# temudschin/xfemm

Measured on AMD Instinct MI355X. Metric: solved DoF/s (assembly+CG to tol) on 2M-tri magnetostatic, higher is better.
Workload: dtype f64; 1 GPU; configs[2]: synthetic 2000000-tri square-domain magnetostatic, linear mu, tol 1e-08; triangles=2000000, dof_total=1002001, dof_per_gpu=1002001, nnz=7006001, pcg_iters=18, newton_iters=1, pcg=Chronopoulos-Gear + AMG V-cycle, parallelism=single GPU

## Files before the change

### xfemm_amd/csrc/xfk_amg.h

```cpp
#pragma once

#include <hip/hip_runtime.h>

#include <map>
#include <memory>
#include <vector>

#include "xfk_internal.h"
#include "xfk_partition.h"

struct xfk_comm;

namespace xfk {

constexpr int kAmgDenseMax = 2048;
constexpr int kAmgMaxLevels = 16;
constexpr int kAmgDeferSlots = 64;
constexpr int kAmgDeferTotal = kAmgDeferSlots + kAmgDeferSlots / 2;

struct AmgLevel {
    int n = 0;
    long long nnz = 0;
    int ncol_lim = 0;
    int ncol_smooth = 0;
    const int *rowptr = nullptr, *col = nullptr;
    const double *val = nullptr;
    DBuf<int> rowptr_o, col_o;
    DBuf<double> val_o;
    DBuf<double> dinv;
    int nc = 0;
    long long pnnz = 0;
    DBuf<int> prow, pcol, rrow, rcol;
    DBuf<double> pval, rval;
// ... 70 lines not shown
    DBuf<int> cnt, agg1, agg, flag, cursor;
    DBuf<int> ap_row, ap_col;
    DBuf<int> pad_col;
    DBuf<double> pad_val;
    DBuf<double> ap_val;
    DBuf<int> dev_int;
    std::map<int, int> cap_hint;
    std::map<int, int> mis_hint;
    int row_max0 = 0;
    void seed_hints();
    DBuf<int> def_dev;
    int *def_host = nullptr;
    int def_n = 0;
    long long *def_target[kAmgDeferSlots / 2] = {};
    int def_verify[kAmgDeferSlots / 2] = {};
    bool foreign = false;
    std::vector<char> nd_plan;
    size_t nd_tl_n = 0, nd_mask_n = 0;
    int load_hints(hipStream_t s, int n0, long long nnz0);
    void save_hints(int n0, long long nnz0);
    int *host_int = nullptr;
    hipEvent_t ev_host = nullptr;
    DBuf<int> mis_out;
    DBuf<char> cub_tmp;

    bool dist = false;
    int rep_rows = 250000;
    int dense_max = kAmgDenseMax;
    int fold_on = -1;
    int col16 = -1;
    int prec32 = -1;
    int lrep = 0;
    xfk_comm *comm = nullptr;
    int nranks = 1, rank = 0;
    std::vector<int> c0;
    int ncmax = 0;
// ... 10 lines not shown
    int *host_big = nullptr;
    int host_big_n = 0;
    double *part_gam_ = nullptr;
    SideStream side;
    bool time_tail = false;
    std::vector<hipEvent_t> tail_ev;
    std::vector<char> tail_kind;
    int tail_used = 0;
    int tail_begin(hipStream_t s, int kind);
    void tail_end(hipStream_t s, int at);
    int tail_read(double &ms_cycle, int &cycles, double &ms_setup);
    SideStream sw;
    bool sw_used = false, rt_pending = false, fold_pending = false;
    DBuf<int> cnt2;
    DBuf<char> cub_tmp2;

    ~Amg();
    void sync_streams()
    {
        if (side.cs) (void)hipStreamSynchronize(side.cs);
        if (sw.cs) (void)hipStreamSynchronize(sw.cs);
    }
    int setup(hipStream_t s, int n, int ncol_lim, const int *rowptr, const int *col, const double *val,
              long long nnz);
    int setup_dist(hipStream_t s, xfk_comm *comm, const HaloPlan &halo, int n, int nh, const int *rowptr,
                   const int *col, const double *val, long long nnz);
    int vcycle(hipStream_t s, const double *r, double *u, const int *done, double *part_gam = nullptr);
    bool gamma_done = false;
    int refresh(hipStream_t s, bool fold = true);
    int reserve_host();
// ... 21 lines not shown
```

### xfemm_amd/csrc/xfk_amg.hip

```cpp
#include <hipcub/hipcub.hpp>

#include <algorithm>
#include <climits>
#include <cmath>
#include <cstdio>
#include <cstdlib>
#include <cstring>
#include <map>
#include <mutex>
#include <vector>

#include "xfk_amg.h"
#include "xfk_comm.h"
#include "xfk_spmv.h"

namespace xfk {

namespace {


constexpr int kB = 256;
inline int nb(long long n) { return (int)((n + kB - 1) / kB); }

using MisKey = unsigned;
// ... 316 lines not shown
        *undecided = 1;
    }
    if (ROOTS) flag[i] = root;
}


__global__ void k_mis_pack(const int *__restrict__ roots, const int *__restrict__ und, const int *__restrict__ run,
                           int *__restrict__ out)
{
    if (threadIdx.x == 0) {
        out[0] = *roots;
        out[1] = *und;
        out[2] = *run;
    }
}

__global__ void k_pattern_diff(int n, const int *__restrict__ rowptr, const int *__restrict__ col,
                               const int *__restrict__ key, int key_nnz, int *__restrict__ out)
{
    const int t = blockIdx.x * blockDim.x + threadIdx.x;
    bool d = false;
    if (t <= n) d = rowptr[t] != key[t];
    if (t < key_nnz) d = d || col[t] != key[n + 1 + t];
    if (d) out[0] = 1;
}

template <int G>
__device__ __forceinline__ void join_best_key(MisKey &best, int &bk, int &bj)
{
#pragma unroll
// ... 826 lines not shown
        if (l == 0) M[(size_t)q * ld + q] = 1.0;
        return;
    }
    const double sq = sc[q];
    for (int k = rowptr[i] + l; k < rowptr[i + 1]; k += kDsG) {
        const int cj = col[k];
        if (cj >= n) continue;
        const int c = perm ? perm[cj] : cj;
        M[(size_t)q * ld + c] = 0.0 + val[k] * sq * sc[c];
    }
}

template <class V>
__global__ void __launch_bounds__(256) k_dense_unperm(int n, int ld, int ldo, const double *__restrict__ M,
                                                      const double *__restrict__ sc, const int *__restrict__ iperm,
                                                      V *__restrict__ out, double *__restrict__ osc)
{
    __shared__ double t[64][65];
    const int bq = blockIdx.y * 64, br = blockIdx.x * 64;
    for (int k = threadIdx.x; k < 64 * 64; k += 256) {
        const int a = k & 63, b = k >> 6;
        t[a][b] = M[(size_t)(br + b) * ld + bq + a];
    }
    __syncthreads();
    for (int k = threadIdx.x; k < 64 * 64; k += 256) {
        const int a = k >> 6, b = k & 63, q = bq + a, r = br + b;
        const int i = iperm ? iperm[q] : (q < n ? q : -1), j = iperm ? iperm[r] : (r < n ? r : -1);
        if (i >= 0 && j >= 0) out[(size_t)i * ldo + j] = (V)(0.5 * (M[(size_t)q * ld + r] + t[a][b]));
    }
    if (blockIdx.x == 0)
        for (int a = threadIdx.x; a < 64; a += 256) {
            const int q = bq + a, i = iperm ? iperm[q] : (q < n ? q : -1);
            if (i >= 0) osc[i] = sc[q];
        }
// ... 1255 lines not shown
        int *slot = M.def_dev.p + M.def_n;
        int *need = (verify && cap > 16) ? M.def_dev.p + kAmgDeferSlots + M.def_n / 2 : nullptr;
        M.def_verify[M.def_n / 2] = need ? cap : 0;
        AMG_CHECK(M.pad_col.alloc((size_t)nrows * cap));
        AMG_CHECK(M.pad_val.alloc((size_t)nrows * cap));
        AMG_CHECK(ccol.alloc((size_t)std::max(1LL, (long long)nrows * cap)));
        AMG_CHECK(cval.alloc((size_t)std::max(1LL, (long long)nrows * cap)));
        launch_sort(cap, slot, need);
        int rc = scan_only(M, s, M.cnt.p, crow.p, nrows);
        if (rc != XFK_OK) return rc;
        if (nrows > 0)
            launch_compact(s, nrows, cap, crow.p, slab_n, M.pad_col.p, M.pad_val.p, ccol.p, cval.p, slot + 1);
        else
            AMG_CHECK(hipMemsetAsync(slot + 1, 0, sizeof(int), s));
        M.def_target[M.def_n / 2] = &cnnz;
        M.def_n += 2;
        cnnz = (long long)nrows * cap;
        return XFK_OK;
    };
    if (key >= 0) {
        auto hint = M.cap_hint.find(key);
        if (hint != M.cap_hint.end()) {
            if (defer && M.def_n + 2 <= kAmgDeferSlots) return deferred_pass(hint->second, M.foreign);
            if (M.foreign) {
                M.cap_hint.erase(hint);
                hint = M.cap_hint.end();
            }
        }
        if (hint != M.cap_hint.end()) {
            bool overflow = false;
// ... 374 lines not shown
    static const bool v = [] {
        const char *e = std::getenv("XFK_NO_SPEC");
        return !(e && std::atoi(e) != 0);
    }();
    return v;
}

bool overlap_enabled()
{
    const char *n = std::getenv("XFK_NO_OVERLAP");
    if (n && std::atoi(n) != 0) return false;
    const char *e = std::getenv("XFK_OVERLAP");
    return e && std::atoi(e) != 0;
}

int Amg::resolve_deferred(hipStream_t s, bool &overflow)
{
    int rc = fetch_deferred(s);
    if (rc != XFK_OK) return rc;
    return wait_deferred(s, overflow);
}

int Amg::fetch_deferred(hipStream_t s)
{
    if (def_n == 0) return XFK_OK;
    AMG_CHECK(hipMemcpyAsync(def_host, def_dev.p, sizeof(int) * kAmgDeferTotal, hipMemcpyDeviceToHost, s));
    AMG_CHECK(hipEventRecord(ev_host, s));
    return XFK_OK;
}

int Amg::wait_deferred(hipStream_t s, bool &overflow)
{
    overflow = false;
    if (def_n == 0) return XFK_OK;
    AMG_CHECK(hipEventSynchronize(ev_host));
    for (int q = 0; q < def_n / 2; ++q) {
        if (def_host[2 * q]) overflow = true;
        else if (def_verify[q] && !def_host[kAmgDeferSlots + q]) overflow = true;
        else *def_target[q] = def_host[2 * q + 1];
        def_verify[q] = 0;
    }
    def_n = 0;
    AMG_CHECK(hipMemsetAsync(def_dev.p, 0, sizeof(int) * kAmgDeferTotal, s));
    return XFK_OK;
}

int Amg::host_ints(int count)
{
    if (host_big_n >= count) return XFK_OK;
    pinned_free(host_big);
    host_big = nullptr;
    host_big_n = 0;
    AMG_CHECK(pinned_malloc((void **)&host_big, sizeof(int) * std::max(count, 1)));
    host_big_n = count;
    return XFK_OK;
}

int Amg::reserve_host()
// ... 8 lines not shown
    }
    constexpr size_t kStage = 64 << 10;
    if (nd_stage_n < kStage) {
        pinned_free(nd_stage);
        nd_stage = nullptr;
        nd_stage_n = 0;
        AMG_CHECK(pinned_malloc((void **)&nd_stage, kStage));
        nd_stage_n = kStage;
    }
    return XFK_OK;
}

int Amg::init(hipStream_t s)
{
    if (!host_int) AMG_CHECK(pinned_malloc((void **)&host_int, 16 * sizeof(int)));
    if (!ev_host) AMG_CHECK(hipEventCreateWithFlags(&ev_host, hipEventDisableTiming));
    if (!def_host) AMG_CHECK(pinned_malloc((void **)&def_host, kAmgDeferTotal * sizeof(int)));
    AMG_CHECK(dev_int.alloc(8));
    AMG_CHECK(def_dev.alloc(kAmgDeferTotal));
    def_n = 0;
    for (int &v : def_verify) v = 0;
    AMG_CHECK(rho.alloc(2 * kAmgMaxLevels));
    k_setup_zero<<<1, 64, 0, s>>>(def_dev.p, kAmgDeferTotal, rho.p, 2 * kAmgMaxLevels);
    if (L.empty()) L.emplace_back(new AmgLevel());
    for (auto &lv : L) {
        lv->dist = false;
        lv->has16 = false;
        lv->has32 = false;
        lv->plan = HaloPlan();
        lv->ts.B = 0;
// ... 154 lines not shown
        save_hints(n0, nnz0);
    }
    return rc;
}

static bool rt_tile_on()
{
    static const bool v = [] {
        const char *e = std::getenv("XFK_RT_TILE");
        return !(e && std::atoi(e) == 0);
    }();
    return v;
}

static int transpose_csr(DBuf<int> &cnt, DBuf<char> &tmp, hipStream_t s, int n, int nc, const int *mrow,
                         const int *mcol, const double *mval, int *trow, int *tcol, double *tval)
{
    AMG_CHECK(cnt.alloc((size_t)std::max(n, nc) + 1));
    AMG_CHECK(hipMemsetAsync(cnt.p, 0, sizeof(int) * ((size_t)nc + 1), s));
    const bool tiled = rt_tile_on();
    if (n > 0) {
        if (tiled) k_rt_tile<false><<<nb(n), 256, 0, s>>>(n, mrow, mcol, mval, trow, cnt.p, tcol, tval);
        else k_rt_count<<<nb(n), kB, 0, s>>>(n, mrow, mcol, cnt.p);
    }
    int rc = scan_only(tmp, s, cnt.p, trow, nc);
    if (rc != XFK_OK) return rc;
    if (tiled) {
        if (n > 0) k_rt_tile<true><<<nb(n), 256, 0, s>>>(n, mrow, mcol, mval, trow, cnt.p, tcol, tval);
        if (nc > 0) k_rt_sort_pairs<<<(int)((((long long)nc + 3) / 4 * 64 + 255) / 256), 256, 0, s>>>(nc, trow, tcol, tval);
        AMG_CHECK(hipGetLastError());
        return XFK_OK;
    }
    if (n > 0) k_rt_fill<<<nb(n), kB, 0, s>>>(n, mrow, mcol, trow, cnt.p, tcol);
    if (nc > 0)
        k_rt_sort_vals<<<(int)(((long long)nc * 64 + 255) / 256), 256, 0, s>>>(nc, trow, tcol, mrow, mcol, mval, tval);
    AMG_CHECK(hipGetLastError());
    return XFK_OK;
}

template <int B>
static int build_col16(hipStream_t st, int n, const int *rowptr, const int *col, long long nnz,
                       DBuf<unsigned short> &c16, DBuf<int> &base)
{
    const int nt = (n + B - 1) / B;
    AMG_CHECK(c16.alloc((size_t)std::max(1LL, nnz)));
    AMG_CHECK(base.alloc((size_t)std::max(1, nt)));
    if (nt > 0) k_tile_col16<B><<<nt, 256, 0, st>>>(n, rowptr, col, c16.p, base.p);
// ... 39 lines not shown
                else
                    k_mis_update<4><<<nb(4LL * n), kB, 0, s>>>(n, A.rowptr, cv, sflag.p, t1.p, key.p, prev, cur,
                                                                nullptr, xc);
            } else {
                k_mis_max<1><<<nb(n), kB, 0, s>>>(n, A.rowptr, cv, sflag.p, key.p, t1.p, prev, cur, run, act.p, xc);
                if (last)
                    k_mis_update<1, true><<<nb(n), kB, 0, s>>>(n, A.rowptr, cv, sflag.p, t1.p, key.p, prev, cur,
                                                                flag.p, xc);
                else
                    k_mis_update<1><<<nb(n), kB, 0, s>>>(n, A.rowptr, cv, sflag.p, t1.p, key.p, prev, cur, nullptr,
                                                          xc);
            }
        }
        int rc = scan_only(*this, s, flag.p, cursor.p, n);
        if (rc != XFK_OK) return rc;
        k_mis_pack<<<1, 64, 0, s>>>(cursor.p + n, und2 + ((rounds - 1) & 1), run, mis_out.p);
        AMG_CHECK(hipMemcpyAsync(host_int + 8, mis_out.p, 3 * sizeof(int), hipMemcpyDeviceToHost, s));
        AMG_CHECK(hipEventRecord(ev_host, s));
        joined = spec;
        if (spec && (rc = joins_and_p()) != XFK_OK) return rc;
        AMG_CHECK(hipEventSynchronize(ev_host));
        if (!host_int[9]) break;
        joined = false;
        if (rounds > 4096) {
            set_error("AMG: MIS-2 aggregation did not terminate");
            return XFK_ERR_NOCONV;
        }
    }
    mis_hint[l] = host_int[10];
    nc = host_int[8];
    stats.mis_rounds[l] = host_int[10];
    int rc = XFK_OK;
// ... 5 lines not shown
    A.nc = (int)nc;
    if (std::getenv("XFK_AMG_DEBUG")) std::fprintf(stderr, "[amg] level %d P nnz %lld\n", l, A.pnnz);
    AMG_CHECK(A.rrow.alloc((size_t)nc + 1));
    AMG_CHECK(A.rcol.alloc((size_t)std::max(1LL, A.pnnz)));
    AMG_CHECK(A.rval.alloc((size_t)std::max(1LL, A.pnnz)));
    const bool off = side_setup_on() && !A.dist && !dist;
    hipStream_t ts = s;
    if (off) {
        if ((rc = sw.init()) != XFK_OK) return rc;
        AMG_CHECK(hipEventRecord(sw.a, s));
        AMG_CHECK(hipStreamWaitEvent(sw.cs, sw.a, 0));
        ts = sw.cs;
        sw_used = true;
    }
    if ((rc = transpose_csr(off ? cnt2 : cnt, off ? cub_tmp2 : cub_tmp, ts, n, (int)nc, A.prow.p, A.pcol.p,
                            A.pval.p, A.rrow.p, A.rcol.p, A.rval.p)) != XFK_OK)
        return rc;
    if (off) {
        AMG_CHECK(hipEventRecord(sw.b, sw.cs));
        rt_pending = true;
    }
    if (l == 0 && A.has16 && (rc = build_col16<256>(ts, (int)nc, A.rrow.p, A.rcol.p, A.pnnz, A.r16, A.r16b)) != XFK_OK)
        return rc;
    if (l == 0 && A.has32 &&
        ((rc = to_f32(ts, (int)nc, A.rrow.p, A.pnnz, A.rval.p, A.r32)) != XFK_OK ||
         (f32_sweep_on() && (rc = to_f32(ts, n, A.rowptr, A.nnz, A.val, A.a32)) != XFK_OK)))
        return rc;
    if (l == 0 && A.has32 && A.dist &&
        ((rc = to_f32(ts, n, A.prow.p, A.pnnz, A.pval.p, A.p32)) != XFK_OK ||
         (rc = build_col16<256>(ts, n, A.prow.p, A.pcol.p, A.pnnz, A.p16, A.p16b)) != XFK_OK))
        return rc;
// ... 315 lines not shown
        st.nn = 1;
        st.nx[0] = 0;
        st.Dn[0] = Db(0, 0);
        st.Rn[0] = Rb(0, 0);
        st.Cn[0] = Cb(0, 0);
        k_bgj_init<<<1 + 2 * nbk, 256, 0, s>>>(nbk, ld, cinv.p, st, maxd, bgj_inv_mode());
        for (int k = 0; k < nbk; ++k) {
            const int p = k & 1, q = (k + 1) & 1;
            k_bgj_step<<<nbk * nbk, 256, 0, s>>>(k, nbk, ld, cinv.p, Db(0, p), Rb(0, p), Cb(0, p), Db(0, q),
                                                 Rb(0, q), Cb(0, q), maxd, bgj_inv_mode());
        }
    }
    {
        const int ldo = ((C.n + kBj - 1) / kBj) * kBj;
        const dim3 g(ld / 64, ld / 64);
        AMG_CHECK(cinv_sc.alloc((size_t)ldo));
        cinv_f64 = !(prec32 < 0 ? f32_on() : prec32 != 0);
        if (cinv_f64) {
            AMG_CHECK(cinv_o64.alloc((size_t)ldo * ldo));
            AMG_CHECK(hipMemsetAsync(cinv_o64.p, 0, sizeof(double) * (size_t)ldo * ldo, s));
            k_dense_unperm<double><<<g, 256, 0, s>>>(C.n, ld, ldo, cinv.p, sc, nd ? cinv_iperm.p : nullptr,
                                                     cinv_o64.p, cinv_sc.p);
        } else {
            AMG_CHECK(cinv_o.alloc((size_t)ldo * ldo));
            AMG_CHECK(hipMemsetAsync(cinv_o.p, 0, sizeof(float) * (size_t)ldo * ldo, s));
            k_dense_unperm<float><<<g, 256, 0, s>>>(C.n, ld, ldo, cinv.p, sc, nd ? cinv_iperm.p : nullptr, cinv_o.p,
                                                    cinv_sc.p);
        }
        cinv_apply = cinv_o.p;
        cinv_ld = ldo;
    }
    return XFK_OK;
}

int Amg::alloc_vectors()
{
    for (int k = 0; k < nlev; ++k) {
        AmgLevel &A = *L[k];
        const size_t nv = (size_t)std::max(1, std::max(A.n, A.ncol_smooth));
        AMG_CHECK(A.xa.alloc(nv));
        AMG_CHECK(A.xb.alloc(nv));
        AMG_CHECK(A.r.alloc((size_t)std::max(1, A.n)));
// ... 39 lines not shown
        k_max_reduce<<<1, kMaxReduceT, 0, s>>>(nb_str(n), rho_part.p, omega, rho.p + 2 * l);
        if (g_prof) g_prof->end();
        if (l == kAmgMaxLevels - 1) break;
        long long nc = 0;
        int rc = aggregate(s, l, nc, true);
        if (rc != XFK_OK) return rc;
        if (nc == 0) break;
        SgX XA{A.rowptr, A.col, A.val, A.ncol_lim, nullptr, nullptr, nullptr, A.has16 ? A.a16.p : nullptr,
               A.has16 ? A.a16b.p : nullptr};
        SgY YP{A.prow.p, A.pcol.p, A.pval.p, nullptr};
        if (fold_pending) {
            AMG_CHECK(hipStreamWaitEvent(s, sw.c, 0));
            fold_pending = false;
        }
        if (g_prof) g_prof->begin(lv + "SpGEMM A P", 0.0);
        rc = spgemm<false>(*this, s, n, XA, YP, A.ftrow, ap_col, ap_val, ap_nnz, 4 * l + 1);
        if (g_prof) g_prof->end();
        if (rc != XFK_OK) return rc;
        if ((int)L.size() <= l + 1) L.emplace_back(new AmgLevel());
        AmgLevel &C = *L[l + 1];
        SgX XR{A.rrow.p, A.rcol.p, A.rval.p, INT_MAX, nullptr, nullptr, nullptr};
        SgY YAP{A.ftrow.p, ap_col.p, ap_val.p, nullptr};
        if (rt_pending) {
            AMG_CHECK(hipStreamWaitEvent(s, sw.b, 0));
            rt_pending = false;
        }
        if (g_prof) g_prof->begin(lv + "SpGEMM R (A P)", 0.0);
        rc = spgemm<false>(*this, s, (int)nc, XR, YAP, C.rowptr_o, C.col_o, C.val_o, C.nnz, 4 * l + 2);
        if (g_prof) g_prof->end();
        if (rc != XFK_OK) return rc;
        A.fold = (fold_on < 0 ? fold_levels() : fold_on != 0) && sweeps == 1 && !A.dist;
// ... 20 lines not shown
            }
            if (n > 0)
                k_fold_p<<<(int)(((long long)n * kFoldLanes + 255) / 256), 256, 0, fs>>>(
                    n, rho.p + 2 * l, A.dinv.p, A.ftrow.p, ap_col.p, ap_val.p, A.prow.p, A.pcol.p, A.pval.p, A.ftcol.p,
                    A.ftval.p);
            if (l == 0 && A.has16 &&
                (rc = build_col16<kCgBlock>(fs, n, A.ftrow.p, A.ftcol.p, ap_nnz, A.f16, A.f16b)) != XFK_OK)
                return rc;
            if (l == 0 && A.has32 && (rc = to_f32(fs, n, A.ftrow.p, ap_nnz, A.ftval.p, A.f32v)) != XFK_OK) return rc;
            if (off) {
                AMG_CHECK(hipEventRecord(sw.c, sw.cs));
                fold_pending = true;
            }
            if (l > 0)
                rc = transpose_csr(off ? cnt2 : cnt, off ? cub_tmp2 : cub_tmp, fs, n, (int)nc, A.ftrow.p, A.ftcol.p,
                                   A.ftval.p, A.frrow.p, A.frcol.p, A.frval.p);
            if (rc != XFK_OK) return rc;
            if (def_n > 0 && def_n + 2 <= kAmgDeferSlots) {
                AMG_CHECK(hipMemcpyAsync(def_dev.p + def_n + 1, A.ftrow.p + n, sizeof(int), hipMemcpyDeviceToDevice, s));
                def_target[def_n / 2] = &A.fnnz;
                def_n += 2;
            } else if (def_n > 0) {
                int len = 0;
                AMG_CHECK(hipMemcpyAsync(&len, A.ftrow.p + n, sizeof(int), hipMemcpyDeviceToHost, s));
                AMG_CHECK(hipStreamSynchronize(s));
                A.fnnz = len;
            }
            if (g_prof) g_prof->end();
        }
        C.n = (int)nc;
        C.ncol_lim = (int)nc;
        C.ncol_smooth = (int)nc;
        C.rowptr = C.rowptr_o.p;
        C.col = C.col_o.p;
        C.val = C.val_o.p;
    }
    nlev = l + 1;
    {
        AmgLevel &C = *L[nlev - 1];
        const bool nd_spec = dense_coarse && spec_on() && !g_prof && def_n > 0 && nlev - 1 > l0 &&
                             C.n >= 8 * kBj && nd_key_n == C.n && C.col == C.col_o.p &&
                             (size_t)nd_key_nnz <= C.col_o.n && !std::getenv("XFK_NO_ND");
        if (nd_spec) {
            AMG_CHECK(mis_out.alloc(4));
            AMG_CHECK(hipMemsetAsync(mis_out.p + 3, 0, sizeof(int), s));
            const int nt = (int)std::max((long long)C.n + 1, nd_key_nnz);
            k_pattern_diff<<<nb(nt), kB, 0, s>>>(C.n, C.rowptr, C.col, nd_key_dev.p, (int)nd_key_nnz, mis_out.p + 3);
            AMG_CHECK(hipMemcpyAsync(host_int + 11, mis_out.p + 3, sizeof(int), hipMemcpyDeviceToHost, s));
        }
        int rc = fetch_deferred(s);
        if (rc != XFK_OK) return rc;
        if (nd_spec) {
            rc = alloc_vectors();
            if (rc != XFK_OK) return rc;
            nd_phases = nd_phases_key;
            if ((rc = dense_inverse(s, C, nd_ld)) != XFK_OK) return rc;
        }
        bool overflow = false;
        rc = wait_deferred(s, overflow);
        if (rc != XFK_OK) return rc;
        if (overflow) {
            if (sw_used) {
                AMG_CHECK(hipStreamSynchronize(sw.cs));
                sw_used = rt_pending = fold_pending = false;
            }
            cap_hint.clear();
            return build(s, l0);
        }
        for (int k = l0; k < nlev; ++k) stats.nnz[k] = L[k]->nnz;
        if (std::getenv("XFK_AMG_HINTS_PRINT")) {
            std::fprintf(stderr, "[amg hints] levels %d:", nlev);
            for (auto &h : cap_hint) std::fprintf(stderr, " cap[%d.%d]=%d", h.first / 4, h.first % 4, h.second);
            for (auto &h : mis_hint) std::fprintf(stderr, " mis[%d]=%d", h.first, h.second);
            for (int k = 0; k < nlev; ++k) std::fprintf(stderr, " n%d=%d/%lld", k, L[k]->n, L[k]->nnz);
            std::fprintf(stderr, "\n");
// ... 893 lines not shown
```

### xfemm_amd/csrc/xfk_api.hip

```cpp
#include <hipcub/hipcub.hpp>

#include "xfk_amg.h"
#include "xfk_spmv.h"

#include <algorithm>
#include <atomic>
#include <chrono>
#include <cmath>
#include <cstring>
#include <map>
#include <mutex>
#include <iterator>
#include <set>
#include <type_traits>
#include <unordered_map>

#include "xfk_age.h"
#include "xfk_comm.h"
#include "xfk_kernels.h"
#include "xfk_magdir.h"
#include <cstdio>
#include <cstdlib>
#include "xfk_partition.h"

// ... 817 lines not shown
        void *tmp = nullptr;
        size_t bytes = 0;
        XFK_CHECK(hipcub::DeviceRadixSort::SortPairs(tmp, bytes, P->color.p, T.keys_out, T.iota, P->perm.p, NE, 0,
                                                     8, s));
        XFK_CHECK(cub_scratch(P, bytes, &tmp));
        XFK_CHECK(hipcub::DeviceRadixSort::SortPairs(tmp, bytes, P->color.p, T.keys_out, T.iota, P->perm.p, NE, 0,
                                                     8, s));
    }
    XFK_CHECK(P->erec.alloc(NE));
    XFK_CHECK(P->ebits.alloc(NE));
    XFK_CHECK(P->slot.alloc(9 * (size_t)NE));
    launch_build_erec(s, NE, P->perm.p, P->p_raw.p, P->lbl_raw.p, P->ebits_raw.p, P->erec.p, P->ebits.p, T.iperm);
    launch_build_slots(s, NE, N, P->p_raw.p, T.iperm, P->rowptr.p, P->col.p, P->slot.p, T.cnt);
    }

    launch_mark_fix_adj(s, N, P->rowptr.p, P->col.p, P->fixed.p, T.flag);
    XFK_CHECK(P->fix_cols_row.alloc(N));
    launch_compact_flags(s, N, T.flag, T.cnt + 1, P->fix_cols_row.p);
    if (P->harmonic) {
        XFK_CHECK(hipMemcpyAsync(P->hpin + 2, T.cnt, sizeof(int) * 2, hipMemcpyDeviceToHost, s));
        XFK_CHECK(hipStreamSynchronize(s));
        const int hc[2] = {P->hpin[2], P->hpin[3]};
        XFK_REQUIRE(hc[0] == 0, XFK_ERR_HIP, "internal: element slot missing from the CSR pattern");
        P->nfix_cols = hc[1];
    } else {
        XFK_CHECK(P->nfix_dev.alloc(1));
        XFK_CHECK(hipMemcpyAsync(P->nfix_dev.p, T.cnt + 1, sizeof(int), hipMemcpyDeviceToDevice, s));
        P->nfix_cols = -1;
    }
    XFK_CHECK(P->mu1.alloc(NE));
    XFK_CHECK(P->mu2.alloc(NE));
    if (!P->harmonic) {
        XFK_CHECK(P->mu1b.alloc(NE));
        XFK_CHECK(P->mu2b.alloc(NE));
        if (P->any_nonlinear && !P->axi) {
            XFK_CHECK(P->dv_el.alloc(NE));
            XFK_CHECK(P->on_el.alloc(NE));
        }
        XFK_CHECK(P->asm_miss.alloc(1));
        XFK_CHECK(hipMemsetAsync(P->asm_miss.p, 0, sizeof(int), s));
        P->miss_checked = false;
    }

    P->age_n = 0;
    if (!P->age_key.empty()) {
        std::vector<int> rc;
        std::vector<double> v;
        for (size_t m = 0; m < P->age_key.size(); ++m) {
            const int r = (int)(P->age_key[m] >> 32), c = (int)(P->age_key[m] & 0xffffffff);
            rc.push_back(r); rc.push_back(c); v.push_back(P->age_val[m]);
            if (r != c) { rc.push_back(c); rc.push_back(r); v.push_back(P->age_val[m]); }
        }
        const int na = (int)v.size();
        DBuf<int> d_rc;
        XFK_CHECK(upload(d_rc, rc.data(), rc.size(), s));
// ... 98 lines not shown
        XFK_CHECK(upload(P->pa_ptr, ptr.data(), ptr.size(), s));
        XFK_CHECK(upload(P->pa_w, w.data(), w.size(), s));
        XFK_CHECK(P->pa_tmp.alloc(nd));
        std::vector<int> chk(nd), chk2(ns);
        XFK_CHECK(d2h(chk.data(), P->pa_dst.p, sizeof(int) * nd, s));
        if (ns) XFK_CHECK(d2h(chk2.data(), P->pa_src.p, sizeof(int) * ns, s));
        for (int v : chk) XFK_REQUIRE(v >= 0, XFK_ERR_HIP, "internal: auxiliary periodic map slot missing");
        for (int v : chk2) XFK_REQUIRE(v >= 0, XFK_ERR_HIP, "internal: auxiliary periodic map source slot missing");
        P->pa_n = nd;
    }

    for (DBuf<double> *v : {&P->b, &P->P, &P->dinv}) XFK_CHECK(v->alloc(N));
    for (DBuf<double> *v : {&P->V, &P->Vold}) XFK_CHECK(v->alloc(NL));
    XFK_CHECK(P->partials.alloc(2 * kRedGrid));
    XFK_CHECK(P->counters.alloc(8));
    XFK_CHECK(hipMemsetAsync(P->counters.p, 0, sizeof(unsigned) * 8, s));
    XFK_CHECK(P->pcg.alloc(1));
    XFK_CHECK(P->nws.alloc(1));
    int rc2 = alloc_cg(P);
    if (rc2 != XFK_OK) return rc2;
    P->symbolic_ready = true;
    return XFK_OK;
}

static int assemble(xfk_problem *P, int iter)
{
    hipStream_t s = P->stream;
    AssembleArgs A = {};
    A.erec = P->erec.p;
    A.ebits = P->ebits.p;
    A.slot = P->slot.p;
// ... 1889 lines not shown
```

### xfemm_amd/csrc/xfk_device.hip

```cpp
#include "xfk_kernels.h"
#include "xfk_axi.h"
#include "xfk_spmv.h"

namespace xfk {


__device__ __forceinline__ double wave_sum(double v)
{
#pragma unroll
    for (int off = 32; off > 0; off >>= 1) v += __shfl_xor(v, off, 64);
    return v;
}

__device__ __forceinline__ double block_sum(double v, double *lds)
{
    v = wave_sum(v);
    const int lane = threadIdx.x & 63, wid = threadIdx.x >> 6;
    __syncthreads();
    if (lane == 0) lds[wid] = v;
    __syncthreads();
    double r = 0.0;
    if (threadIdx.x == 0) {
        const int nw = (blockDim.x + 63) >> 6;
        for (int w = 0; w < nw; ++w) r += lds[w];
// ... 571 lines not shown
            dst[3 * j + q] = s[q];
        }
    }
    if (missing) atomicAdd(bad, 1);
}

__global__ void k_lookup_slots(int n, const int *__restrict__ rc, const int *__restrict__ rowptr,
                               const int *__restrict__ col, int *__restrict__ out)
{
    int i = blockIdx.x * blockDim.x + threadIdx.x;
    if (i >= n) return;
    out[i] = find_slot(rowptr, col, rc[2 * i], rc[2 * i + 1]);
}

__global__ void k_mark_fix_adj(int N, const int *__restrict__ rowptr, const int *__restrict__ col,
                               const unsigned char *__restrict__ fixed, int *__restrict__ flag)
{
    int r = blockIdx.x * blockDim.x + threadIdx.x;
    if (r >= N) return;
    int f = 0;
    if (!fixed[r])
        for (int k = rowptr[r]; k < rowptr[r + 1]; ++k) f |= fixed[col[k]];
    flag[r] = f;
}

__global__ void k_compact_flags(int N, const int *__restrict__ flag, int *__restrict__ cursor,
                                int *__restrict__ out)
{
    int r = blockIdx.x * blockDim.x + threadIdx.x;
    if (r >= N || !flag[r]) return;
    out[atomicAdd(cursor, 1)] = r;
}

// ... 656 lines not shown
void launch_build_erec(hipStream_t s, int NE, const int *perm, const int *p, const int *lbl, const int *ebits_raw,
                       int4 *erec, int *ebits, int *iperm)
{
    if (NE) k_build_erec<<<nblk(NE), kBlock, 0, s>>>(NE, perm, p, lbl, ebits_raw, erec, ebits, iperm);
}
void launch_build_slots(hipStream_t s, int NE, int nrows, const int *p, const int *iperm, const int *rowptr,
                        const int *col, int *slot, int *bad)
{
    if (NE) k_build_slots<<<nblk(NE), kBlock, 0, s>>>(NE, nrows, p, iperm, rowptr, col, slot, bad);
}
void launch_lookup_slots(hipStream_t s, int n, const int *rc, const int *rowptr, const int *col, int *out)
{
    if (n) k_lookup_slots<<<nblk(n), kBlock, 0, s>>>(n, rc, rowptr, col, out);
}
void launch_mark_fix_adj(hipStream_t s, int N, const int *rowptr, const int *col, const unsigned char *fixed,
                         int *flag)
{
    if (N) k_mark_fix_adj<<<nblk(N), kBlock, 0, s>>>(N, rowptr, col, fixed, flag);
}
void launch_compact_flags(hipStream_t s, int N, const int *flag, int *cursor, int *out)
{
    if (N) k_compact_flags<<<nblk(N), kBlock, 0, s>>>(N, flag, cursor, out);
}
void launch_assemble_rows(hipStream_t s, int N, const AssembleArgs &A)
{
    if (N <= 0) return;
    const int g = (N + kRowBlock - 1) / kRowBlock;
    static const bool xcd = [] {
        const char *e = std::getenv("XFK_ASM_XCD");
        return !(e && std::atoi(e) == 0);
    }();
    if (!xcd && !A.axi) {
        if (A.iter == 0) k_assemble_rows<false, true, false><<<g, kRowBlock, 0, s>>>(N, A);
// ... 72 lines not shown
```

### xfemm_amd/csrc/xfk_internal.h

```cpp
#pragma once

#include <hip/hip_runtime.h>

#include <algorithm>
#include <cstdint>
#include <map>
#include <string>
#include <unordered_map>
#include <thread>
#include <vector>

#include "../../include/xfemm_kernels.h"
#include "xfk_partition.h"

struct xfk_comm;

namespace xfk {

struct Amg;

constexpr int kBlock = 256;
constexpr int kRedGrid = 1024;
constexpr double kPI = 3.141592653589793238462643383;
constexpr double kDEG = 0.01745329251994329576923690768;
// ... 225 lines not shown
hipError_t warm_module_postproc();
hipError_t warm_module_sort();
void stream_release(hipStream_t s);
void stream_pool_drain();
int sort_elements_device(hipStream_t s, int n, const unsigned *score_dev, int *perm_dev, unsigned long long *key,
                         unsigned long long *tmp, unsigned long long *red, unsigned long long *cin, int *flag,
                         int *passes);
long long stream_pool_idle();
struct SideStream {
    hipStream_t cs = nullptr;
    hipEvent_t a = nullptr, b = nullptr, c = nullptr;
    int init();
    ~SideStream();
};
bool overlap_enabled();
template <class Ex, class In, class Bd>
int exchange_overlapped(hipStream_t s, SideStream &ss, Ex &&exch, In &&interior, Bd &&boundary)
{
    XFK_CHECK(hipEventRecord(ss.a, s));
    XFK_CHECK(hipStreamWaitEvent(ss.cs, ss.a, 0));
    const int rc = exch(ss.cs);
    if (rc != XFK_OK) return rc;
    XFK_CHECK(hipEventRecord(ss.b, ss.cs));
    interior();
    XFK_CHECK(hipStreamWaitEvent(s, ss.b, 0));
    boundary();
    return XFK_OK;
}

}
// ... 332 lines not shown
```

### xfemm_amd/csrc/xfk_kernels.h

```cpp
#pragma once

#include "xfk_internal.h"

namespace xfk {

struct AssembleArgs {
    const int4 *erec;
    const int *ebits;
    const int *slot;
    const double *x, *y;
    const DevLabel *labels;
    const DevBlock *blocks;
    const DevLine *lines;
    const DevCirc *circs;
    const double *bhB, *bhH, *bhS;
    double *mu1, *mu2;
    const double *V;
    double *val, *b;
    int iter;
    int axi;
    double ext_ro, ext_ri, ext_zo;
    const int *p_raw, *lbl_raw, *ebits_raw, *n2e_ptr, *n2e, *rowptr, *col;
    double *mu1_out, *mu2_out;
    int *miss;
// ... 46 lines not shown
void launch_row_copy(hipStream_t s, int N, const int *p, const int *n2e_ptr, const int *n2e, const int *fill_ptr,
                     const int *fill_col, const int *tmp, const int *rowptr, int *col, int *diag);
void launch_jp_round(hipStream_t s, int N, int NE, int round, unsigned char *active, int *pending_round,
                     const int *p, const int *n2e_ptr, const int *n2e, int *color, unsigned long long *maxkey,
                     unsigned long long *used);
void launch_color_hist(hipStream_t s, int NE, const int *color, int *hist, int maxc);
void launch_iota(hipStream_t s, int n, int *a);
void launch_build_erec(hipStream_t s, int NE, const int *perm, const int *p, const int *lbl, const int *ebits_raw,
                       int4 *erec, int *ebits, int *iperm);
void launch_build_slots(hipStream_t s, int NE, int nrows, const int *p, const int *iperm, const int *rowptr,
                        const int *col, int *slot, int *bad);
void launch_add_at_slots(hipStream_t s, int n, const int *slot, const double *v, double *data);
void launch_lookup_slots(hipStream_t s, int n, const int *rc, const int *rowptr, const int *col, int *out);
void launch_mark_fix_adj(hipStream_t s, int N, const int *rowptr, const int *col, const unsigned char *fixed,
                         int *flag);
void launch_compact_flags(hipStream_t s, int N, const int *flag, int *cursor, int *out);
void launch_assemble_rows(hipStream_t s, int N, const AssembleArgs &A);
void launch_point_currents(hipStream_t s, int n, const int *nodes, const double *J, double *b);
void launch_dirichlet(hipStream_t s, int nrows, const int *rows, int nadj, const int *nadj_dev, int nadj_max,
                      const int *adj, const int *rowptr, const int *col, const int *diag, const unsigned char *fixed,
                      const double *fix_first, const double *fix_last, double *val, double *b);
void launch_map(hipStream_t s, int n, const int *dst, const int *ptr, const int *src, const double *w,
                double *data, double *tmp);
void launch_diag_inv(hipStream_t s, int N, const int *diag, const double *val, double *dinv, CgState *S);
void launch_newton_res(hipStream_t s, int N, const double *V, const double *Vold, double *partials,
                       unsigned *counter, NewtonScalars *S);
void launch_relax(hipStream_t s, int N, double relax, double *V, const double *Vold);
void launch_scale(hipStream_t s, int N, double sc, const double *V, double *out);

}
// ... 1 lines not shown
```

Before: 189.2 million DoF/s.

## Trim memsets and copies from the AMG setup and assembly launch chain

Adds a default-on XFK_LEAN_CHAIN mode that removes small memsets and memcpys from the stream. The MIS pack kernel writes straight into mapped pinned host memory. The pattern-diff flag rides along with the deferred-readback buffer, and the dense-inverse padding is zeroed inside the unpermute kernel instead of a full memset. The transpose counter memset is skipped when the buffer is known clean, deferred fnnz reuses an earlier slot, and the fix-adjacency kernel zeroes the counters. The aim is to cut launch and API overhead in setup, at the cost of relying on buffer-cleanliness invariants that could go stale.

```diff
diff --git a/xfemm_amd/csrc/xfk_amg.h b/xfemm_amd/csrc/xfk_amg.h
--- a/xfemm_amd/csrc/xfk_amg.h
+++ b/xfemm_amd/csrc/xfk_amg.h
@@ -16,7 +16,8 @@
 constexpr int kAmgDenseMax = 2048;
 constexpr int kAmgMaxLevels = 16;
 constexpr int kAmgDeferSlots = 64;
-constexpr int kAmgDeferTotal = kAmgDeferSlots + kAmgDeferSlots / 2;
+constexpr int kAmgDeferNd = kAmgDeferSlots + kAmgDeferSlots / 2;
+constexpr int kAmgDeferTotal = kAmgDeferNd + 1;
 
 struct AmgLevel {
     int n = 0;
@@ -117,12 +118,14 @@
     int def_n = 0;
     long long *def_target[kAmgDeferSlots / 2] = {};
     int def_verify[kAmgDeferSlots / 2] = {};
+    int def_src[kAmgDeferSlots / 2] = {};
     bool foreign = false;
     std::vector<char> nd_plan;
     size_t nd_tl_n = 0, nd_mask_n = 0;
     int load_hints(hipStream_t s, int n0, long long nnz0);
     void save_hints(int n0, long long nnz0);
     int *host_int = nullptr;
+    int *host_int_dev = nullptr;
     hipEvent_t ev_host = nullptr;
     DBuf<int> mis_out;
     DBuf<char> cub_tmp;
@@ -163,6 +166,8 @@
     bool sw_used = false, rt_pending = false, fold_pending = false;
     DBuf<int> cnt2;
     DBuf<char> cub_tmp2;
+    size_t rt_clean = 0;
+    int *rt_clean_p = nullptr;
 
     ~Amg();
     void sync_streams()
diff --git a/xfemm_amd/csrc/xfk_amg.hip b/xfemm_amd/csrc/xfk_amg.hip
--- a/xfemm_amd/csrc/xfk_amg.hip
+++ b/xfemm_amd/csrc/xfk_amg.hip
@@ -354,6 +354,20 @@
         out[2] = *run;
     }
 }
+__global__ void k_mis_pack_host(const int *__restrict__ roots, const int *__restrict__ und,
+                                const int *__restrict__ run, int *__restrict__ out, int *__restrict__ host)
+{
+    if (threadIdx.x == 0) {
+        const int a = *roots, b = *und, c = *run;
+        out[0] = a;
+        out[1] = b;
+        out[2] = c;
+        host[0] = a;
+        host[1] = b;
+        host[2] = c;
+        __threadfence_system();
+    }
+}
 
 __global__ void k_pattern_diff(int n, const int *__restrict__ rowptr, const int *__restrict__ col,
                                const int *__restrict__ key, int key_nnz, int *__restrict__ out)
@@ -1210,10 +1224,18 @@
 template <class V>
 __global__ void __launch_bounds__(256) k_dense_unperm(int n, int ld, int ldo, const double *__restrict__ M,
                                                       const double *__restrict__ sc, const int *__restrict__ iperm,
-                                                      V *__restrict__ out, double *__restrict__ osc)
+                                                      V *__restrict__ out, double *__restrict__ osc, bool pad)
 {
     __shared__ double t[64][65];
     const int bq = blockIdx.y * 64, br = blockIdx.x * 64;
+    if (pad) {
+        const long long np = ldo - n, tot = np * ldo + (long long)n * np;
+        const long long nthr = (long long)gridDim.x * gridDim.y * 256;
+        for (long long k = ((long long)blockIdx.y * gridDim.x + blockIdx.x) * 256 + threadIdx.x; k < tot; k += nthr) {
+            if (k < np * ldo) out[(size_t)n * ldo + k] = (V)0;
+            else out[(size_t)((k - np * ldo) / np) * ldo + n + (k - np * ldo) % np] = (V)0;
+        }
+    }
     for (int k = threadIdx.x; k < 64 * 64; k += 256) {
         const int a = k & 63, b = k >> 6;
         t[a][b] = M[(size_t)(br + b) * ld + bq + a];
@@ -2499,6 +2521,7 @@
         else
             AMG_CHECK(hipMemsetAsync(slot + 1, 0, sizeof(int), s));
         M.def_target[M.def_n / 2] = &cnnz;
+        M.def_src[M.def_n / 2] = M.def_n / 2;
         M.def_n += 2;
         cnnz = (long long)nrows * cap;
         return XFK_OK;
@@ -2903,6 +2926,15 @@
     return e && std::atoi(e) != 0;
 }
 
+bool lean_chain()
+{
+    static const bool v = [] {
+        const char *e = std::getenv("XFK_LEAN_CHAIN");
+        return !(e && std::atoi(e) == 0);
+    }();
+    return v;
+}
+
 int Amg::resolve_deferred(hipStream_t s, bool &overflow)
 {
     int rc = fetch_deferred(s);
@@ -2926,11 +2958,11 @@
     for (int q = 0; q < def_n / 2; ++q) {
         if (def_host[2 * q]) overflow = true;
         else if (def_verify[q] && !def_host[kAmgDeferSlots + q]) overflow = true;
-        else *def_target[q] = def_host[2 * q + 1];
+        else *def_target[q] = def_host[2 * def_src[q] + 1];
         def_verify[q] = 0;
     }
     def_n = 0;
-    AMG_CHECK(hipMemsetAsync(def_dev.p, 0, sizeof(int) * kAmgDeferTotal, s));
+    if (!lean_chain() || overflow) AMG_CHECK(hipMemsetAsync(def_dev.p, 0, sizeof(int) * kAmgDeferTotal, s));
     return XFK_OK;
 }
 
@@ -2969,6 +3001,7 @@
 int Amg::init(hipStream_t s)
 {
     if (!host_int) AMG_CHECK(pinned_malloc((void **)&host_int, 16 * sizeof(int)));
+    if (!host_int_dev) AMG_CHECK(hipHostGetDevicePointer((void **)&host_int_dev, host_int, 0));
     if (!ev_host) AMG_CHECK(hipEventCreateWithFlags(&ev_host, hipEventDisableTiming));
     if (!def_host) AMG_CHECK(pinned_malloc((void **)&def_host, kAmgDeferTotal * sizeof(int)));
     AMG_CHECK(dev_int.alloc(8));
@@ -3153,11 +3186,15 @@
 }
 
 static int transpose_csr(DBuf<int> &cnt, DBuf<char> &tmp, hipStream_t s, int n, int nc, const int *mrow,
-                         const int *mcol, const double *mval, int *trow, int *tcol, double *tval)
+                         const int *mcol, const double *mval, int *trow, int *tcol, double *tval,
+                         size_t *clean = nullptr, int **clean_p = nullptr)
 {
     AMG_CHECK(cnt.alloc((size_t)std::max(n, nc) + 1));
-    AMG_CHECK(hipMemsetAsync(cnt.p, 0, sizeof(int) * ((size_t)nc + 1), s));
     const bool tiled = rt_tile_on();
+    const bool keep = clean && clean_p && *clean_p == cnt.p && *clean >= (size_t)nc + 1;
+    const size_t was = keep ? *clean : 0;
+    if (!keep) AMG_CHECK(hipMemsetAsync(cnt.p, 0, sizeof(int) * ((size_t)nc + 1), s));
+    if (clean) *clean = 0;
     if (n > 0) {
         if (tiled) k_rt_tile<false><<<nb(n), 256, 0, s>>>(n, mrow, mcol, mval, trow, cnt.p, tcol, tval);
         else k_rt_count<<<nb(n), kB, 0, s>>>(n, mrow, mcol, cnt.p);
@@ -3168,8 +3205,13 @@
         if (n > 0) k_rt_tile<true><<<nb(n), 256, 0, s>>>(n, mrow, mcol, mval, trow, cnt.p, tcol, tval);
         if (nc > 0) k_rt_sort_pairs<<<(int)((((long long)nc + 3) / 4 * 64 + 255) / 256), 256, 0, s>>>(nc, trow, tcol, tval);
         AMG_CHECK(hipGetLastError());
+        if (clean) {
+            *clean = std::max(was, (size_t)nc + 1);
+            *clean_p = cnt.p;
+        }
         return XFK_OK;
     }
+    if (clean) *clean = 0;
     if (n > 0) k_rt_fill<<<nb(n), kB, 0, s>>>(n, mrow, mcol, trow, cnt.p, tcol);
     if (nc > 0)
         k_rt_sort_vals<<<(int)(((long long)nc * 64 + 255) / 256), 256, 0, s>>>(nc, trow, tcol, mrow, mcol, mval, tval);
@@ -3239,8 +3281,13 @@
         }
         int rc = scan_only(*this, s, flag.p, cursor.p, n);
         if (rc != XFK_OK) return rc;
-        k_mis_pack<<<1, 64, 0, s>>>(cursor.p + n, und2 + ((rounds - 1) & 1), run, mis_out.p);
-        AMG_CHECK(hipMemcpyAsync(host_int + 8, mis_out.p, 3 * sizeof(int), hipMemcpyDeviceToHost, s));
+        if (lean_chain()) {
+            k_mis_pack_host<<<1, 64, 0, s>>>(cursor.p + n, und2 + ((rounds - 1) & 1), run, mis_out.p,
+                                             host_int_dev + 8);
+        } else {
+            k_mis_pack<<<1, 64, 0, s>>>(cursor.p + n, und2 + ((rounds - 1) & 1), run, mis_out.p);
+            AMG_CHECK(hipMemcpyAsync(host_int + 8, mis_out.p, 3 * sizeof(int), hipMemcpyDeviceToHost, s));
+        }
         AMG_CHECK(hipEventRecord(ev_host, s));
         joined = spec;
         if (spec && (rc = joins_and_p()) != XFK_OK) return rc;
@@ -3276,7 +3323,8 @@
         sw_used = true;
     }
     if ((rc = transpose_csr(off ? cnt2 : cnt, off ? cub_tmp2 : cub_tmp, ts, n, (int)nc, A.prow.p, A.pcol.p,
-                            A.pval.p, A.rrow.p, A.rcol.p, A.rval.p)) != XFK_OK)
+                            A.pval.p, A.rrow.p, A.rcol.p, A.rval.p, off && lean_chain() ? &rt_clean : nullptr,
+                            &rt_clean_p)) != XFK_OK)
         return rc;
     if (off) {
         AMG_CHECK(hipEventRecord(sw.b, sw.cs));
@@ -3622,18 +3670,19 @@
     {
         const int ldo = ((C.n + kBj - 1) / kBj) * kBj;
         const dim3 g(ld / 64, ld / 64);
+        const bool lean = lean_chain();
         AMG_CHECK(cinv_sc.alloc((size_t)ldo));
         cinv_f64 = !(prec32 < 0 ? f32_on() : prec32 != 0);
         if (cinv_f64) {
             AMG_CHECK(cinv_o64.alloc((size_t)ldo * ldo));
-            AMG_CHECK(hipMemsetAsync(cinv_o64.p, 0, sizeof(double) * (size_t)ldo * ldo, s));
+            if (!lean) AMG_CHECK(hipMemsetAsync(cinv_o64.p, 0, sizeof(double) * (size_t)ldo * ldo, s));
             k_dense_unperm<double><<<g, 256, 0, s>>>(C.n, ld, ldo, cinv.p, sc, nd ? cinv_iperm.p : nullptr,
-                                                     cinv_o64.p, cinv_sc.p);
+                                                     cinv_o64.p, cinv_sc.p, lean);
         } else {
             AMG_CHECK(cinv_o.alloc((size_t)ldo * ldo));
-            AMG_CHECK(hipMemsetAsync(cinv_o.p, 0, sizeof(float) * (size_t)ldo * ldo, s));
+            if (!lean) AMG_CHECK(hipMemsetAsync(cinv_o.p, 0, sizeof(float) * (size_t)ldo * ldo, s));
             k_dense_unperm<float><<<g, 256, 0, s>>>(C.n, ld, ldo, cinv.p, sc, nd ? cinv_iperm.p : nullptr, cinv_o.p,
-                                                    cinv_sc.p);
+                                                    cinv_sc.p, lean);
         }
         cinv_apply = cinv_o.p;
         cinv_ld = ldo;
@@ -3703,7 +3752,9 @@
             fold_pending = false;
         }
         if (g_prof) g_prof->begin(lv + "SpGEMM A P", 0.0);
+        const int ap_def = def_n;
         rc = spgemm<false>(*this, s, n, XA, YP, A.ftrow, ap_col, ap_val, ap_nnz, 4 * l + 1);
+        const bool ap_deferred = rc == XFK_OK && def_n == ap_def + 2;
         if (g_prof) g_prof->end();
         if (rc != XFK_OK) return rc;
         if ((int)L.size() <= l + 1) L.emplace_back(new AmgLevel());
@@ -3754,10 +3805,15 @@
             }
             if (l > 0)
                 rc = transpose_csr(off ? cnt2 : cnt, off ? cub_tmp2 : cub_tmp, fs, n, (int)nc, A.ftrow.p, A.ftcol.p,
-                                   A.ftval.p, A.frrow.p, A.frcol.p, A.frval.p);
+                                   A.ftval.p, A.frrow.p, A.frcol.p, A.frval.p,
+                                   off && lean_chain() ? &rt_clean : nullptr, &rt_clean_p);
             if (rc != XFK_OK) return rc;
             if (def_n > 0 && def_n + 2 <= kAmgDeferSlots) {
-                AMG_CHECK(hipMemcpyAsync(def_dev.p + def_n + 1, A.ftrow.p + n, sizeof(int), hipMemcpyDeviceToDevice, s));
+                def_src[def_n / 2] = def_n / 2;
+                if (lean_chain() && ap_deferred) def_src[def_n / 2] = ap_def / 2;
+                else
+                    AMG_CHECK(hipMemcpyAsync(def_dev.p + def_n + 1, A.ftrow.p + n, sizeof(int),
+                                             hipMemcpyDeviceToDevice, s));
                 def_target[def_n / 2] = &A.fnnz;
                 def_n += 2;
             } else if (def_n > 0) {
@@ -3781,12 +3837,18 @@
         const bool nd_spec = dense_coarse && spec_on() && !g_prof && def_n > 0 && nlev - 1 > l0 &&
                              C.n >= 8 * kBj && nd_key_n == C.n && C.col == C.col_o.p &&
                              (size_t)nd_key_nnz <= C.col_o.n && !std::getenv("XFK_NO_ND");
+        const bool lean = lean_chain();
         if (nd_spec) {
-            AMG_CHECK(mis_out.alloc(4));
-            AMG_CHECK(hipMemsetAsync(mis_out.p + 3, 0, sizeof(int), s));
             const int nt = (int)std::max((long long)C.n + 1, nd_key_nnz);
-            k_pattern_diff<<<nb(nt), kB, 0, s>>>(C.n, C.rowptr, C.col, nd_key_dev.p, (int)nd_key_nnz, mis_out.p + 3);
-            AMG_CHECK(hipMemcpyAsync(host_int + 11, mis_out.p + 3, sizeof(int), hipMemcpyDeviceToHost, s));
+            if (lean) {
+                k_pattern_diff<<<nb(nt), kB, 0, s>>>(C.n, C.rowptr, C.col, nd_key_dev.p, (int)nd_key_nnz,
+                                                     def_dev.p + kAmgDeferNd);
+            } else {
+                AMG_CHECK(mis_out.alloc(4));
+                AMG_CHECK(hipMemsetAsync(mis_out.p + 3, 0, sizeof(int), s));
+                k_pattern_diff<<<nb(nt), kB, 0, s>>>(C.n, C.rowptr, C.col, nd_key_dev.p, (int)nd_key_nnz, mis_out.p + 3);
+                AMG_CHECK(hipMemcpyAsync(host_int + 11, mis_out.p + 3, sizeof(int), hipMemcpyDeviceToHost, s));
+            }
         }
         int rc = fetch_deferred(s);
         if (rc != XFK_OK) return rc;
@@ -3799,6 +3861,7 @@
         bool overflow = false;
         rc = wait_deferred(s, overflow);
         if (rc != XFK_OK) return rc;
+        if (nd_spec && lean) host_int[11] = def_host[kAmgDeferNd];
         if (overflow) {
             if (sw_used) {
                 AMG_CHECK(hipStreamSynchronize(sw.cs));
diff --git a/xfemm_amd/csrc/xfk_api.hip b/xfemm_amd/csrc/xfk_api.hip
--- a/xfemm_amd/csrc/xfk_api.hip
+++ b/xfemm_amd/csrc/xfk_api.hip
@@ -855,9 +855,18 @@
     launch_build_slots(s, NE, N, P->p_raw.p, T.iperm, P->rowptr.p, P->col.p, P->slot.p, T.cnt);
     }
 
-    launch_mark_fix_adj(s, N, P->rowptr.p, P->col.p, P->fixed.p, T.flag);
+    const bool lean = lean_chain() && !P->harmonic && N > 0;
+    if (lean) {
+        XFK_CHECK(P->nfix_dev.alloc(1));
+        XFK_CHECK(P->asm_miss.alloc(1));
+        XFK_CHECK(P->counters.alloc(8));
+        launch_mark_fix_adj(s, N, P->rowptr.p, P->col.p, P->fixed.p, T.flag, P->nfix_dev.p, P->asm_miss.p,
+                            P->counters.p);
+    } else {
+        launch_mark_fix_adj(s, N, P->rowptr.p, P->col.p, P->fixed.p, T.flag);
+    }
     XFK_CHECK(P->fix_cols_row.alloc(N));
-    launch_compact_flags(s, N, T.flag, T.cnt + 1, P->fix_cols_row.p);
+    launch_compact_flags(s, N, T.flag, lean ? P->nfix_dev.p : T.cnt + 1, P->fix_cols_row.p);
     if (P->harmonic) {
         XFK_CHECK(hipMemcpyAsync(P->hpin + 2, T.cnt, sizeof(int) * 2, hipMemcpyDeviceToHost, s));
         XFK_CHECK(hipStreamSynchronize(s));
@@ -866,7 +875,7 @@
         P->nfix_cols = hc[1];
     } else {
         XFK_CHECK(P->nfix_dev.alloc(1));
-        XFK_CHECK(hipMemcpyAsync(P->nfix_dev.p, T.cnt + 1, sizeof(int), hipMemcpyDeviceToDevice, s));
+        if (!lean) XFK_CHECK(hipMemcpyAsync(P->nfix_dev.p, T.cnt + 1, sizeof(int), hipMemcpyDeviceToDevice, s));
         P->nfix_cols = -1;
     }
     XFK_CHECK(P->mu1.alloc(NE));
@@ -879,7 +888,7 @@
             XFK_CHECK(P->on_el.alloc(NE));
         }
         XFK_CHECK(P->asm_miss.alloc(1));
-        XFK_CHECK(hipMemsetAsync(P->asm_miss.p, 0, sizeof(int), s));
+        if (!lean) XFK_CHECK(hipMemsetAsync(P->asm_miss.p, 0, sizeof(int), s));
         P->miss_checked = false;
     }
 
@@ -1008,7 +1017,7 @@
     for (DBuf<double> *v : {&P->V, &P->Vold}) XFK_CHECK(v->alloc(NL));
     XFK_CHECK(P->partials.alloc(2 * kRedGrid));
     XFK_CHECK(P->counters.alloc(8));
-    XFK_CHECK(hipMemsetAsync(P->counters.p, 0, sizeof(unsigned) * 8, s));
+    if (!lean) XFK_CHECK(hipMemsetAsync(P->counters.p, 0, sizeof(unsigned) * 8, s));
     XFK_CHECK(P->pcg.alloc(1));
     XFK_CHECK(P->nws.alloc(1));
     int rc2 = alloc_cg(P);
diff --git a/xfemm_amd/csrc/xfk_device.hip b/xfemm_amd/csrc/xfk_device.hip
--- a/xfemm_amd/csrc/xfk_device.hip
+++ b/xfemm_amd/csrc/xfk_device.hip
@@ -609,9 +609,15 @@
 }
 
 __global__ void k_mark_fix_adj(int N, const int *__restrict__ rowptr, const int *__restrict__ col,
-                               const unsigned char *__restrict__ fixed, int *__restrict__ flag)
+                               const unsigned char *__restrict__ fixed, int *__restrict__ flag,
+                               int *__restrict__ z1a, int *__restrict__ z1b, unsigned *__restrict__ z8)
 {
     int r = blockIdx.x * blockDim.x + threadIdx.x;
+    if (blockIdx.x == 0 && threadIdx.x < 8) {
+        if (threadIdx.x == 0 && z1a) *z1a = 0;
+        if (threadIdx.x == 0 && z1b) *z1b = 0;
+        if (z8) z8[threadIdx.x] = 0u;
+    }
     if (r >= N) return;
     int f = 0;
     if (!fixed[r])
@@ -1298,9 +1304,14 @@
     if (n) k_lookup_slots<<<nblk(n), kBlock, 0, s>>>(n, rc, rowptr, col, out);
 }
 void launch_mark_fix_adj(hipStream_t s, int N, const int *rowptr, const int *col, const unsigned char *fixed,
+                         int *flag, int *z1a, int *z1b, unsigned *z8)
+{
+    if (N) k_mark_fix_adj<<<nblk(N), kBlock, 0, s>>>(N, rowptr, col, fixed, flag, z1a, z1b, z8);
+}
+void launch_mark_fix_adj(hipStream_t s, int N, const int *rowptr, const int *col, const unsigned char *fixed,
                          int *flag)
 {
-    if (N) k_mark_fix_adj<<<nblk(N), kBlock, 0, s>>>(N, rowptr, col, fixed, flag);
+    if (N) k_mark_fix_adj<<<nblk(N), kBlock, 0, s>>>(N, rowptr, col, fixed, flag, nullptr, nullptr, nullptr);
 }
 void launch_compact_flags(hipStream_t s, int N, const int *flag, int *cursor, int *out)
 {
diff --git a/xfemm_amd/csrc/xfk_internal.h b/xfemm_amd/csrc/xfk_internal.h
--- a/xfemm_amd/csrc/xfk_internal.h
+++ b/xfemm_amd/csrc/xfk_internal.h
@@ -263,6 +263,7 @@
     ~SideStream();
 };
 bool overlap_enabled();
+bool lean_chain();
 template <class Ex, class In, class Bd>
 int exchange_overlapped(hipStream_t s, SideStream &ss, Ex &&exch, In &&interior, Bd &&boundary)
 {
diff --git a/xfemm_amd/csrc/xfk_kernels.h b/xfemm_amd/csrc/xfk_kernels.h
--- a/xfemm_amd/csrc/xfk_kernels.h
+++ b/xfemm_amd/csrc/xfk_kernels.h
@@ -84,6 +84,8 @@
 void launch_lookup_slots(hipStream_t s, int n, const int *rc, const int *rowptr, const int *col, int *out);
 void launch_mark_fix_adj(hipStream_t s, int N, const int *rowptr, const int *col, const unsigned char *fixed,
                          int *flag);
+void launch_mark_fix_adj(hipStream_t s, int N, const int *rowptr, const int *col, const unsigned char *fixed,
+                         int *flag, int *z1a, int *z1b, unsigned *z8);
 void launch_compact_flags(hipStream_t s, int N, const int *flag, int *cursor, int *out);
 void launch_assemble_rows(hipStream_t s, int N, const AssembleArgs &A);
 void launch_point_currents(hipStream_t s, int n, const int *nodes, const double *J, double *b);
```

New measurement: 190.2 million DoF/s (median of 6 runs). No clear change (+0.5%).
